# lewisjared/rscm

Hardware: AMD Instinct MI355X
Metric: ensemble-member-years/sec, two-layer 1750-2500 f64 (higher is better)
Workload: dtype f64

## Files before the change

### rscm_amd/csrc/two_layer.hip

```cpp
#include "two_layer_body.hpp"

namespace rscm {

namespace {

__device__ unsigned long long g_guard_counts[tl::kGuardKinds];

template <int MODE, bool LDS, bool STORE>
__global__ __launch_bounds__(kBlock) void two_layer_kernel(TwoLayerArgs a)
{
    extern __shared__ double lds_forcing[];
    if constexpr (LDS) {
        const int32_t len = a.step_end - a.step_begin;
        const int32_t total = a.n_scen * len;
        for (int32_t idx = threadIdx.x; idx < total; idx += kBlock) {
            const int32_t s = idx / len, k = idx - s * len;
            lds_forcing[idx] = a.forcing[(size_t)s * a.n_times + a.step_begin + a.src_off + k];
        }
        __syncthreads();
    }
    const int64_t i = (int64_t)blockIdx.x * kBlock + threadIdx.x;
    if (i >= a.n_members) return;
    const int32_t guard = tl::two_layer_body<MODE, LDS, STORE>(a, lds_forcing, i, a.step_begin, a.step_end);
    if constexpr (MODE == 0) {
        if (a.count_guards && (threadIdx.x & 63) == 0) atomicAdd(&g_guard_counts[guard], 1ull);
    }
}

template <int MODE, bool LDS>
__global__ __launch_bounds__(kBlock) void two_layer_ref_kernel(TwoLayerArgs a, TwoLayerRefArgs r)
{
    extern __shared__ double lds_forcing[];
    if constexpr (LDS) {
        const int32_t len = a.step_end - a.step_begin;
        const int32_t total = a.n_scen * len;
        for (int32_t idx = threadIdx.x; idx < total; idx += kBlock) {
            const int32_t s = idx / len, k = idx - s * len;
            lds_forcing[idx] = a.forcing[(size_t)s * a.n_times + a.step_begin + a.src_off + k];
        }
        __syncthreads();
    }
    const int64_t i = (int64_t)blockIdx.x * kBlock + threadIdx.x;
    if (i >= a.n_members) return;
    const int32_t guard = tl::two_layer_body<MODE, LDS, false, NoCache, true>(a, lds_forcing, i, a.step_begin, a.step_end, NoCache(), &r);
    if constexpr (MODE == 0) {
        if (a.count_guards && (threadIdx.x & 63) == 0) atomicAdd(&g_guard_counts[guard], 1ull);
    }
}

}


template <bool STORE>
static hipError_t launch_impl(const TwoLayerArgs& a, int mode, hipStream_t s)
{
    if (a.n_members <= 0) return hipSuccess;
    if (STORE && a.step_end <= a.step_begin) return hipSuccess;
    const size_t lds = a.lds_forcing ? (size_t)a.n_scen * (a.step_end - a.step_begin) * sizeof(double) : 0;
    const dim3 grid((unsigned)((a.n_members + kBlock - 1) / kBlock));
    void (*kern)(TwoLayerArgs) =
        mode == 0 ? (a.lds_forcing ? two_layer_kernel<0, true, STORE> : two_layer_kernel<0, false, STORE>)
                  : (a.lds_forcing ? two_layer_kernel<1, true, STORE> : two_layer_kernel<1, false, STORE>);
    if (lds > (size_t)kMaxStaticLds) {
        hipError_t e = hipFuncSetAttribute(reinterpret_cast<const void*>(kern),
                                           hipFuncAttributeMaxDynamicSharedMemorySize, (int)lds);
        if (e != hipSuccess) return e;
    }
    hipLaunchKernelGGL(kern, grid, dim3(kBlock), lds, s, a);
    return hipGetLastError();
}

hipError_t launch_two_layer(const TwoLayerArgs& a, int mode, hipStream_t s)
{
    return launch_impl<true>(a, mode, s);
}

hipError_t launch_two_layer_loglik(const TwoLayerArgs& a, int mode, hipStream_t s)
{
    return launch_impl<false>(a, mode, s);
}

hipError_t launch_two_layer_loglik_ref(const TwoLayerArgs& a, const TwoLayerRefArgs& r, int mode, hipStream_t s)
{
    if (a.n_members <= 0) return hipSuccess;
    const size_t lds = a.lds_forcing ? (size_t)a.n_scen * (a.step_end - a.step_begin) * sizeof(double) : 0;
    const dim3 grid((unsigned)((a.n_members + kBlock - 1) / kBlock));
    void (*kern)(TwoLayerArgs, TwoLayerRefArgs) =
        mode == 0 ? (a.lds_forcing ? two_layer_ref_kernel<0, true> : two_layer_ref_kernel<0, false>)
                  : (a.lds_forcing ? two_layer_ref_kernel<1, true> : two_layer_ref_kernel<1, false>);
    if (lds > (size_t)kMaxStaticLds) {
        hipError_t e = hipFuncSetAttribute(reinterpret_cast<const void*>(kern),
                                           hipFuncAttributeMaxDynamicSharedMemorySize, (int)lds);
        if (e != hipSuccess) return e;
    }
    hipLaunchKernelGGL(kern, grid, dim3(kBlock), lds, s, a, r);
    return hipGetLastError();
}

hipError_t two_layer_guard_counts(int64_t* out)
{
    unsigned long long c[tl::kGuardKinds] = {};
    hipError_t e = hipDeviceSynchronize();
    if (e == hipSuccess && out) e = hipMemcpyFromSymbol(c, HIP_SYMBOL(g_guard_counts), sizeof c);
    if (e != hipSuccess) return e;
    if (out)
        for (int k = 0; k < tl::kGuardKinds; ++k) out[k] = (int64_t)c[k];
    const unsigned long long zero[tl::kGuardKinds] = {};
    return hipMemcpyToSymbol(HIP_SYMBOL(g_guard_counts), zero, sizeof zero);
}

}
```

### rscm_amd/csrc/two_layer_body.hpp

```cpp
#pragma once

#include <type_traits>

#include "rk4_device.hpp"
#include "rscm_device.hpp"
#include "two_layer_box.hpp"
#include "two_layer_chunk_box.hpp"

namespace rscm {
namespace tl {

struct TLConst {
    double lambda0, a, eff_eta, eta, cs, cd, rcs, rcd;
};

template <bool SPEC, bool TAGS = SPEC>
__device__ __forceinline__ void rhs_exact(const TLConst& p, double erf, double ts, double td,
                                          double& dts, double& dtd, int32_t& acc)
{
    const double diff = ts - td;
    const double lambda_eff = p.lambda0 - p.a * ts;
    const double hx_s = p.eff_eta * diff;
    const double num_s = erf - lambda_eff * ts - hx_s;
    const double num_d = p.eta * diff;
    if constexpr (SPEC) {
        dts = spec_div(num_s, p.cs, p.rcs);
        dtd = spec_div(num_d, p.cd, p.rcd);
        if constexpr (TAGS) acc = max3_i32(acc, window_tag(num_s), window_tag(num_d));
    } else {
        dts = num_s / p.cs;
        dtd = num_d / p.cd;
    }
}

template <bool SPEC, bool TAGS = SPEC>
__device__ __forceinline__ void rk4_step_exact(const TLConst& p, double erf, double h,
                                               double half_step, double sixth, double& ts,
                                               double& td, int32_t& acc)
{
    double k1s, k1d, k2s, k2d, k3s, k3d, k4s, k4d;
    rhs_exact<SPEC, TAGS>(p, erf, ts, td, k1s, k1d, acc);
    rhs_exact<SPEC, TAGS>(p, erf, ts + k1s * half_step, td + k1d * half_step, k2s, k2d, acc);
    rhs_exact<SPEC, TAGS>(p, erf, ts + k2s * half_step, td + k2d * half_step, k3s, k3d, acc);
    rhs_exact<SPEC, TAGS>(p, erf, ts + k3s * h, td + k3d * h, k4s, k4d, acc);
    if constexpr (SPEC) {
        ts = rk4_combine_fused2(ts, k1s, k2s, k3s, k4s, sixth);
        td = rk4_combine_fused2(td, k1d, k2d, k3d, k4d, sixth);
    } else {
        ts = rk4_combine(ts, k1s, k2s, k3s, k4s, sixth);
        td = rk4_combine(td, k1d, k2d, k3d, k4d, sixth);
    }
}

namespace box {

constexpr double pow2(int e)
{
    double r = 1.0;
    for (; e > 0; --e) r *= 2.0;
    for (; e < 0; ++e) r *= 0.5;
    return r;
}

static_assert(kCsLo >= -128 && kCsHi <= 129 && kCdLo >= -128 && kCdHi <= 129, "heat-capacity boxes must lie in the divisor window");

constexpr uint32_t neg_edge(int lo) { return 0u - ((uint32_t)(1023 + lo) << 21); }
constexpr uint32_t span(int lo, int hi) { return (uint32_t)(hi - lo) << 21; }

__device__ __forceinline__ bool positive_in(double x, int lo, int hi)
{
    return x >= pow2(lo) && x < pow2(hi);
}

template <int lo = kForcingLo, int hi = kForcingHi>
__device__ __forceinline__ bool forcing_in(double f)
{
    return (__double_as_longlong(f) == 0) | (box_tag(f, neg_edge(lo)) < span(lo, hi));
}

__device__ __forceinline__ bool params_in(const TLConst& p, double h, double half_step)
{
    return positive_in(p.lambda0, kLambda0Lo, kLambda0Hi) &&
           (__double_as_longlong(p.a) == 0 || positive_in(p.a, kALo, kAHi)) &&
           positive_in(p.eff_eta, kEffEtaLo, kEffEtaHi) && positive_in(p.eta, kEtaLo, kEtaHi) &&
           positive_in(p.cs, kCsLo, kCsHi) && positive_in(p.cd, kCdLo, kCdHi) &&
           positive_in(h, kHLo, kHHi) && positive_in(half_step, kHLo, kHHi);
}

}

namespace chunk {

static_assert(kWideDivLo >= box::kCsLo && kWideDivHi <= box::kCdHi && kCsLo >= kWideDivLo && kCsHi <= kWideDivHi &&
                  kCdLo >= kWideDivLo && kCdHi <= kWideDivHi,
              "the chunk's heat capacities must lie in the wide window's divisor box");

__device__ __forceinline__ bool params_in(const TLConst& p, double h, double half_step, double sixth)
{
    using box::positive_in;
    return positive_in(p.lambda0, kLambda0Lo, kLambda0Hi) &&
           (__double_as_longlong(p.a) == 0 || positive_in(p.a, kALo, kAHi)) &&
           positive_in(p.eff_eta, kEffEtaLo, kEffEtaHi) && positive_in(p.eta, kEtaLo, kEtaHi) &&
           positive_in(p.cs, kCsLo, kCsHi) && positive_in(p.cd, kCdLo, kCdHi) &&
           positive_in(h, kHLo, kHHi) && positive_in(half_step, kHalfLo, kHalfHi) && positive_in(sixth, kSixthLo, kSixthHi);
}

}

constexpr int32_t kUnrolledSubSteps = 10;

struct TLFast {
    double l0, a, ee, ed;
};

__device__ __forceinline__ void rhs_fast(const TLFast& p, double erf_cs, double ts, double w, double& dts, double& dw)
{
    const double q = __builtin_fma(p.a, ts, -p.l0);
    const double t = __builtin_fma(q, ts, erf_cs);
    dts = __builtin_fma(-p.ee, w, t);
    dw = __builtin_fma(-p.ed, w, dts);
}

__device__ __forceinline__ void rk4_year_fast(const TLFast& p, double erf_cs, int32_t m, double h, double half_step, double third,
                                              double sixth, double& ts, double& td)
{
    double w = ts - td;
    for (int32_t s = 0; s < m; ++s) {
        double k1s, k1w, k2s, k2w, k3s, k3w, k4s, k4w;
        rhs_fast(p, erf_cs, ts, w, k1s, k1w);
        rhs_fast(p, erf_cs, __builtin_fma(k1s, half_step, ts), __builtin_fma(k1w, half_step, w), k2s, k2w);
        rhs_fast(p, erf_cs, __builtin_fma(k2s, half_step, ts), __builtin_fma(k2w, half_step, w), k3s, k3w);
        rhs_fast(p, erf_cs, __builtin_fma(k3s, h, ts), __builtin_fma(k3w, h, w), k4s, k4w);
        ts = __builtin_fma(k2s + k3s, third, __builtin_fma(k1s + k4s, sixth, ts));
        w = __builtin_fma(k2w + k3w, third, __builtin_fma(k1w + k4w, sixth, w));
    }
    td = ts - w;
}

__device__ __forceinline__ TLFast make_fast(double lambda0, double a, double efficacy, double eta, double cs, double cd, double& inv_cs)
{
    inv_cs = 1.0 / cs;
    TLFast p;
    p.l0 = lambda0 * inv_cs;
    p.a = a * inv_cs;
    p.ee = efficacy * eta * inv_cs;
    p.ed = eta / cd;
    return p;
}

struct LikAcc {
    double part_s = 0.0, part_d = 0.0;
    bool bad = false;
    int32_t oi = 0;
};

__device__ __forceinline__ void lik_consume(const TwoLayerArgs& a, LikAcc& L, int32_t row, double ts,
                                            double td)
{
    while (L.oi < a.n_obs && a.obs_tidx[L.oi] == row) {
        const bool deep = a.obs_is_deep[L.oi] != 0;
        const double m = deep ? td : ts;
        if (!is_finite(m)) L.bad = true;
        const double sigma = a.obs_sigma[L.oi];
        const double residual = a.obs_value[L.oi] - m;
        const double chi = (residual * residual) / (sigma * sigma);
        double l = -0.5 * chi;
        if (a.normalize) {
            l -= 0.5 * 1.8378770664093453;
            l -= log(sigma);
        }
        if (deep) L.part_d += l;
        else L.part_s += l;
        ++L.oi;
    }
}

struct LikRef {
    double sum_s = -0.0, sum_d = -0.0, b_s = 0.0, b_d = 0.0;
    bool have_s = false, have_d = false;
};

__device__ __forceinline__ double lik_term(const TwoLayerArgs& a, int32_t k, double m)
{
    const double sigma = a.obs_sigma[k];
    const double residual = a.obs_value[k] - m;
    const double chi = (residual * residual) / (sigma * sigma);
    double l = -0.5 * chi;
    if (a.normalize) {
        l -= 0.5 * 1.8378770664093453;
        l -= log(sigma);
    }
    return l;
}

__device__ __forceinline__ void lik_settle(const TwoLayerArgs& a, const TwoLayerRefArgs& r, LikAcc& L, bool deep, double sum, int32_t count,
                                           double& b, double& part, int64_t i, int64_t N)
{
    b = sum / (double)count;
    if (!is_finite(b)) L.bad = true;
    for (int32_t k = 0; k < L.oi; ++k) {
        const int32_t slot = r.obs_slot[k];
        if ((a.obs_is_deep[k] != 0) != deep || slot < 0) continue;
        part += lik_term(a, k, r.defer[(size_t)slot * N + i] - b);
    }
}

__device__ __forceinline__ void lik_consume_ref(const TwoLayerArgs& a, const TwoLayerRefArgs& r, LikAcc& L, LikRef& R, int32_t row,
                                                double ts, double td, int64_t i, int64_t N)
{
    auto reference_row = [&](int32_t v) {
        return r.on[v] && row >= r.begin[v] && row <= r.last[v] && (r.stride[v] == 1 || (row - r.begin[v]) % r.stride[v] == 0);
    };
    if (reference_row(0)) R.sum_s += ts;
    if (reference_row(1)) R.sum_d += td;
    while (L.oi < a.n_obs && a.obs_tidx[L.oi] == row) {
        const bool deep = a.obs_is_deep[L.oi] != 0;
        const double m = deep ? td : ts;
        if (!is_finite(m)) L.bad = true;
        const int32_t slot = r.obs_slot[L.oi];
        if (slot >= 0) {
            r.defer[(size_t)slot * N + i] = m;
        } else {
            const bool anomaly = deep ? r.on[1] != 0 : r.on[0] != 0;
            const double l = lik_term(a, L.oi, anomaly ? m - (deep ? R.b_d : R.b_s) : m);
            if (deep) L.part_d += l;
            else L.part_s += l;
        }
        ++L.oi;
    }
    if (r.on[0] && row == r.last[0]) {
        lik_settle(a, r, L, false, R.sum_s, r.count[0], R.b_s, L.part_s, i, N);
        R.have_s = true;
    }
    if (r.on[1] && row == r.last[1]) {
        lik_settle(a, r, L, true, R.sum_d, r.count[1], R.b_d, L.part_d, i, N);
        R.have_d = true;
    }
}

enum : int32_t { kGuardNumerators = 0, kGuardStates = 1, kGuardChunks = 2, kGuardKinds = 3 };

template <int MODE, bool LDS, bool STORE, class Cache = NoCache, bool REF = false>
__device__ __forceinline__ int32_t two_layer_body(const TwoLayerArgs& a, const double* lds_forcing, int64_t i, int32_t step_begin,
                                               int32_t step_end, const Cache& cache = Cache(), const TwoLayerRefArgs* ref = nullptr)
{
    static_assert(!(REF && STORE), "reference periods belong to the fused likelihood");
    const int32_t len = step_end - step_begin;
    const int64_t N = a.row_stride;

    const double lambda0 = cache.param(a.params, a.uniform_rows, 0, N, i);
    const double pa = cache.param(a.params, a.uniform_rows, 1, N, i);
    const double efficacy = cache.param(a.params, a.uniform_rows, 2, N, i);
    const double eta = cache.param(a.params, a.uniform_rows, 3, N, i);
    const double cs = cache.param(a.params, a.uniform_rows, 4, N, i);
    const double cd = cache.param(a.params, a.uniform_rows, 5, N, i);
    const int32_t scen = a.scen ? a.scen[i] : 0;
    const double* fglob = a.link ? a.link + (size_t)a.src_off * N + i : a.forcing + (size_t)scen * a.n_times + a.src_off;
    const size_t fstride = a.link ? (size_t)N : (size_t)1;
    const int32_t fl0 = scen * len - step_begin;
    auto forcing_at = [&](int32_t n) -> double {
        if constexpr (LDS) return lds_forcing[fl0 + n];
        else return fglob[(size_t)n * fstride];
    };
    auto forcing_first = [&]() -> double {
        if constexpr (Cache::kOn) {
            if (a.link && cache.has_link(0)) return cache.link(0);
        }
        return forcing_at(step_begin);
    };
    auto forcing_ahead = [&](int32_t n, int32_t np, double current) -> double {
        if constexpr (Cache::kOn) return n < np ? forcing_at(np) : current;
        else return forcing_at(np);
    };

    double ts = cache.state(0, a.ts + (size_t)step_begin * N + i);
    double td = cache.state(1, a.td + (size_t)step_begin * N + i);
    double* out_ts = a.ts + (size_t)(step_begin + 1) * N + i;
    double* out_td = a.td + (size_t)(step_begin + 1) * N + i;

    const double h = a.h;
    const double half_step = a.h_half;
    const double sixth = a.h_sixth;
    const int32_t last = step_end - 1;

    LikAcc lik;
    [[maybe_unused]] LikRef lik_ref;
    [[maybe_unused]] auto consume = [&](int32_t row) {
        if constexpr (REF) lik_consume_ref(a, *ref, lik, lik_ref, row, ts, td, i, N);
        else lik_consume(a, lik, row, ts, td);
    };
    if constexpr (!STORE) consume(step_begin);

    double erf_next = forcing_first();
    int32_t m_next = a.nsub[step_begin];

    int32_t guard = -1;
    if constexpr (MODE == 0) {
        TLConst p;
        p.lambda0 = lambda0;
        p.a = pa;
        p.eff_eta = efficacy * eta;
        p.eta = eta;
        p.cs = cs;
        p.cd = cd;
        const ConstDiv dcs = make_const_div(cs), dcd = make_const_div(cd);
        p.rcs = dcs.r;
        p.rcd = dcd.r;
        const int32_t acc0 = (dcs.ok && dcd.ok) ? (int32_t)0x80000000 : 0;
        const bool guard_states = __all(!a.numerator_guard && box::params_in(p, h, half_step));
        const bool guard_chunks = guard_states && __all(chunk::params_in(p, h, half_step, sixth));
        auto years = [&](auto guard) {
            constexpr int32_t kGuard = decltype(guard)::value;
            constexpr bool kStates = kGuard > 0;
            constexpr bool kChunks = kGuard > 1;
            for (int32_t n = step_begin; n < step_end; ++n) {
                const double erf = erf_next;
                const int32_t m = m_next;
                const int32_t np = n < last ? n + 1 : n;
                erf_next = forcing_ahead(n, np, erf_next);
                m_next = a.nsub[np];
                const double ts0 = ts, td0 = td;
                bool replay;
                if constexpr (kStates) {
                    int32_t no_tags = 0;
                    auto sub_step = [&](uint32_t& acc, uint32_t edge, bool tag) {
                        if (tag) acc = max3_u32(acc, box_tag(ts, edge), box_tag(td, edge));
                        rk4_step_exact<true, false>(p, erf, h, half_step, sixth, ts, td, no_tags);
                    };
                    if (kChunks && m == kUnrolledSubSteps) {
                        constexpr uint32_t kEdge = box::neg_edge(chunk::kStateLo), kSpan = box::span(chunk::kStateLo, chunk::kStateHi);
                        uint32_t acc = box::forcing_in<chunk::kForcingLo, chunk::kForcingHi>(erf) ? 0u : ~0u;
#pragma unroll
                        for (int32_t s = 0; s < kUnrolledSubSteps; ++s) sub_step(acc, kEdge, s % kGuard == 0);
                        replay = acc >= kSpan;
                    } else {
                        constexpr uint32_t kEdge = box::neg_edge(box::kStateLo), kSpan = box::span(box::kStateLo, box::kStateHi);
                        uint32_t acc = box::forcing_in(erf) ? 0u : ~0u;
                        if (m == kUnrolledSubSteps) {
#pragma unroll
                            for (int32_t s = 0; s < kUnrolledSubSteps; ++s) sub_step(acc, kEdge, true);
                        } else {
                            for (int32_t s = 0; s < m; ++s) sub_step(acc, kEdge, true);
                        }
                        replay = acc >= kSpan;
                    }
                } else {
                    int32_t acc = acc0;
                    for (int32_t s = 0; s < m; ++s) rk4_step_exact<true>(p, erf, h, half_step, sixth, ts, td, acc);
                    replay = acc >= 0;
                }
                const bool settled = (ts0 != ts0) || (td0 != td0);
                if (__builtin_expect(replay && !settled, 0)) {
                    ts = ts0;
                    td = td0;
                    int32_t unused = 0;
                    for (int32_t s = 0; s < m; ++s) rk4_step_exact<false>(p, erf, h, half_step, sixth, ts, td, unused);
                }
                if constexpr (STORE) {
                    *out_ts = ts;
                    *out_td = td;
                    cache.put(0, ts);
                    cache.put(1, td);
                    out_ts += N;
                    out_td += N;
                } else {
                    consume(n + 1);
                }
            }
        };
        if (guard_chunks) years(std::integral_constant<int32_t, chunk::kChunkSubSteps>());
        else if (guard_states) years(std::integral_constant<int32_t, 1>());
        else years(std::integral_constant<int32_t, 0>());
        guard = guard_chunks ? kGuardChunks : guard_states ? kGuardStates : kGuardNumerators;
    } else {
        double inv_cs;
        const TLFast p = make_fast(lambda0, pa, efficacy, eta, cs, cd, inv_cs);
        const double third = h / 3.0;
        for (int32_t n = step_begin; n < step_end; ++n) {
            const double erf = erf_next * inv_cs;
            const int32_t m = m_next;
            const int32_t np = n < last ? n + 1 : n;
            erf_next = forcing_ahead(n, np, erf_next);
            m_next = a.nsub[np];
            rk4_year_fast(p, erf, m, h, half_step, third, sixth, ts, td);
            if constexpr (STORE) {
                *out_ts = ts;
                *out_td = td;
                cache.put(0, ts);
                cache.put(1, td);
                out_ts += N;
                out_td += N;
            } else {
                consume(n + 1);
            }
        }
    }
    if (cache.last_step()) a.status[i] = (is_finite(ts) && is_finite(td)) ? 0 : 1;
    if constexpr (!STORE) {
        if (lik.oi < a.n_obs) lik.bad = true;
        if constexpr (REF) {
            if ((ref->on[0] && !lik_ref.have_s) || (ref->on[1] && !lik_ref.have_d)) lik.bad = true;
        }
        const double total = a.first_is_deep ? (0.0 + lik.part_d) + lik.part_s
                                             : (0.0 + lik.part_s) + lik.part_d;
        a.loglik[i] = lik.bad ? -__builtin_inf() : total;
    }
    return guard;
}

}
}
```

Baseline: 34.99 billion.

## Read uniform forcing via scalar loads and unroll year loop in pairs

When all members share one forcing series, the kernels now skip LDS staging and read forcing and substep counts through scalar (constant address space) loads. The year loop is restructured to process two years per iteration with lookahead prefetch, and adds a lean path that drops the forcing range check once upcoming years are known to be in range. Replay of out-of-box steps becomes wave-uniform via ballot, and output stores use a wave-base pointer plus lane offset. This adds template instantiations and code complexity, and relies on forcing and nsub being safe to read through scalar loads.

Result: no change. 34.95 billion, median of 2 (-0.1%).

```diff
diff --git a/rscm_amd/csrc/two_layer.hip b/rscm_amd/csrc/two_layer.hip
--- a/rscm_amd/csrc/two_layer.hip
+++ b/rscm_amd/csrc/two_layer.hip
@@ -6,22 +6,36 @@
 
 __device__ unsigned long long g_guard_counts[tl::kGuardKinds];
 
+__host__ __device__ inline bool uniform_forcing(const TwoLayerArgs& a)
+{
+    return a.scen == nullptr && a.n_scen == 1 && a.link == nullptr && a.n_times < (1 << 28);
+}
+
+__device__ __forceinline__ void stage_forcing(const TwoLayerArgs& a, double* lds_forcing)
+{
+    const int32_t len = a.step_end - a.step_begin;
+    const int32_t total = a.n_scen * len;
+    for (int32_t idx = threadIdx.x; idx < total; idx += kBlock) {
+        const int32_t s = idx / len, k = idx - s * len;
+        lds_forcing[idx] = a.forcing[(size_t)s * a.n_times + a.step_begin + a.src_off + k];
+    }
+    __syncthreads();
+}
+
 template <int MODE, bool LDS, bool STORE>
 __global__ __launch_bounds__(kBlock) void two_layer_kernel(TwoLayerArgs a)
 {
     extern __shared__ double lds_forcing[];
-    if constexpr (LDS) {
-        const int32_t len = a.step_end - a.step_begin;
-        const int32_t total = a.n_scen * len;
-        for (int32_t idx = threadIdx.x; idx < total; idx += kBlock) {
-            const int32_t s = idx / len, k = idx - s * len;
-            lds_forcing[idx] = a.forcing[(size_t)s * a.n_times + a.step_begin + a.src_off + k];
-        }
-        __syncthreads();
+    const int64_t i = (int64_t)blockIdx.x * kBlock + threadIdx.x;
+    int32_t guard;
+    if (uniform_forcing(a)) {
+        if (i >= a.n_members) return;
+        guard = tl::two_layer_body<MODE, false, STORE, NoCache, false, true>(a, nullptr, i, a.step_begin, a.step_end);
+    } else {
+        if constexpr (LDS) stage_forcing(a, lds_forcing);
+        if (i >= a.n_members) return;
+        guard = tl::two_layer_body<MODE, LDS, STORE>(a, lds_forcing, i, a.step_begin, a.step_end);
     }
-    const int64_t i = (int64_t)blockIdx.x * kBlock + threadIdx.x;
-    if (i >= a.n_members) return;
-    const int32_t guard = tl::two_layer_body<MODE, LDS, STORE>(a, lds_forcing, i, a.step_begin, a.step_end);
     if constexpr (MODE == 0) {
         if (a.count_guards && (threadIdx.x & 63) == 0) atomicAdd(&g_guard_counts[guard], 1ull);
     }
@@ -31,18 +45,16 @@
 __global__ __launch_bounds__(kBlock) void two_layer_ref_kernel(TwoLayerArgs a, TwoLayerRefArgs r)
 {
     extern __shared__ double lds_forcing[];
-    if constexpr (LDS) {
-        const int32_t len = a.step_end - a.step_begin;
-        const int32_t total = a.n_scen * len;
-        for (int32_t idx = threadIdx.x; idx < total; idx += kBlock) {
-            const int32_t s = idx / len, k = idx - s * len;
-            lds_forcing[idx] = a.forcing[(size_t)s * a.n_times + a.step_begin + a.src_off + k];
-        }
-        __syncthreads();
+    const int64_t i = (int64_t)blockIdx.x * kBlock + threadIdx.x;
+    int32_t guard;
+    if (uniform_forcing(a)) {
+        if (i >= a.n_members) return;
+        guard = tl::two_layer_body<MODE, false, false, NoCache, true, true>(a, nullptr, i, a.step_begin, a.step_end, NoCache(), &r);
+    } else {
+        if constexpr (LDS) stage_forcing(a, lds_forcing);
+        if (i >= a.n_members) return;
+        guard = tl::two_layer_body<MODE, LDS, false, NoCache, true>(a, lds_forcing, i, a.step_begin, a.step_end, NoCache(), &r);
     }
-    const int64_t i = (int64_t)blockIdx.x * kBlock + threadIdx.x;
-    if (i >= a.n_members) return;
-    const int32_t guard = tl::two_layer_body<MODE, LDS, false, NoCache, true>(a, lds_forcing, i, a.step_begin, a.step_end, NoCache(), &r);
     if constexpr (MODE == 0) {
         if (a.count_guards && (threadIdx.x & 63) == 0) atomicAdd(&g_guard_counts[guard], 1ull);
     }
@@ -56,7 +68,7 @@
 {
     if (a.n_members <= 0) return hipSuccess;
     if (STORE && a.step_end <= a.step_begin) return hipSuccess;
-    const size_t lds = a.lds_forcing ? (size_t)a.n_scen * (a.step_end - a.step_begin) * sizeof(double) : 0;
+    const size_t lds = (a.lds_forcing && !uniform_forcing(a)) ? (size_t)a.n_scen * (a.step_end - a.step_begin) * sizeof(double) : 0;
     const dim3 grid((unsigned)((a.n_members + kBlock - 1) / kBlock));
     void (*kern)(TwoLayerArgs) =
         mode == 0 ? (a.lds_forcing ? two_layer_kernel<0, true, STORE> : two_layer_kernel<0, false, STORE>)
@@ -83,7 +95,7 @@
 hipError_t launch_two_layer_loglik_ref(const TwoLayerArgs& a, const TwoLayerRefArgs& r, int mode, hipStream_t s)
 {
     if (a.n_members <= 0) return hipSuccess;
-    const size_t lds = a.lds_forcing ? (size_t)a.n_scen * (a.step_end - a.step_begin) * sizeof(double) : 0;
+    const size_t lds = (a.lds_forcing && !uniform_forcing(a)) ? (size_t)a.n_scen * (a.step_end - a.step_begin) * sizeof(double) : 0;
     const dim3 grid((unsigned)((a.n_members + kBlock - 1) / kBlock));
     void (*kern)(TwoLayerArgs, TwoLayerRefArgs) =
         mode == 0 ? (a.lds_forcing ? two_layer_ref_kernel<0, true> : two_layer_ref_kernel<0, false>)
diff --git a/rscm_amd/csrc/two_layer_body.hpp b/rscm_amd/csrc/two_layer_body.hpp
--- a/rscm_amd/csrc/two_layer_body.hpp
+++ b/rscm_amd/csrc/two_layer_body.hpp
@@ -76,6 +76,15 @@
 __device__ __forceinline__ bool forcing_in(double f)
 {
     return (__double_as_longlong(f) == 0) | (box_tag(f, neg_edge(lo)) < span(lo, hi));
+}
+
+template <int lo = kForcingLo, int hi = kForcingHi>
+__device__ __forceinline__ uint32_t forcing_acc_uniform(double f)
+{
+    const uint64_t bits = (uint64_t)__double_as_longlong(f);
+    const uint32_t tag = ((uint32_t)(bits >> 32) << 1) + neg_edge(lo);
+    const uint32_t outside = tag < span(lo, hi) ? 0u : ~0u;
+    return bits == 0 ? 0u : outside;
 }
 
 __device__ __forceinline__ bool params_in(const TLConst& p, double h, double half_step)
@@ -240,11 +249,18 @@
 
 enum : int32_t { kGuardNumerators = 0, kGuardStates = 1, kGuardChunks = 2, kGuardKinds = 3 };
 
-template <int MODE, bool LDS, bool STORE, class Cache = NoCache, bool REF = false>
+__device__ __forceinline__ int64_t first_lane(int64_t v)
+{
+    const uint32_t lo = __builtin_amdgcn_readfirstlane((uint32_t)v), hi = __builtin_amdgcn_readfirstlane((uint32_t)((uint64_t)v >> 32));
+    return (int64_t)(((uint64_t)hi << 32) | lo);
+}
+
+template <int MODE, bool LDS, bool STORE, class Cache = NoCache, bool REF = false, bool UNIFORM = false>
 __device__ __forceinline__ int32_t two_layer_body(const TwoLayerArgs& a, const double* lds_forcing, int64_t i, int32_t step_begin,
                                                int32_t step_end, const Cache& cache = Cache(), const TwoLayerRefArgs* ref = nullptr)
 {
     static_assert(!(REF && STORE), "reference periods belong to the fused likelihood");
+    static_assert(!(UNIFORM && (LDS || Cache::kOn)), "the uniform forcing is read from the table, by the stand-alone kernels");
     const int32_t len = step_end - step_begin;
     const int64_t N = a.row_stride;
 
@@ -254,13 +270,21 @@
     const double eta = cache.param(a.params, a.uniform_rows, 3, N, i);
     const double cs = cache.param(a.params, a.uniform_rows, 4, N, i);
     const double cd = cache.param(a.params, a.uniform_rows, 5, N, i);
-    const int32_t scen = a.scen ? a.scen[i] : 0;
-    const double* fglob = a.link ? a.link + (size_t)a.src_off * N + i : a.forcing + (size_t)scen * a.n_times + a.src_off;
-    const size_t fstride = a.link ? (size_t)N : (size_t)1;
+    const int32_t scen = (!UNIFORM && a.scen) ? a.scen[i] : 0;
+    const double* fglob = (!UNIFORM && a.link) ? a.link + (size_t)a.src_off * N + i : a.forcing + (size_t)scen * a.n_times + a.src_off;
+    const size_t fstride = (!UNIFORM && a.link) ? (size_t)N : (size_t)1;
     const int32_t fl0 = scen * len - step_begin;
+    typedef const __attribute__((address_space(4))) char* scalar_bytes;
+    [[maybe_unused]] const scalar_bytes funi = (scalar_bytes)(uintptr_t)(a.forcing + a.src_off);
+    const scalar_bytes nuni = (scalar_bytes)(uintptr_t)a.nsub;
     auto forcing_at = [&](int32_t n) -> double {
-        if constexpr (LDS) return lds_forcing[fl0 + n];
+        if constexpr (UNIFORM) return *(const volatile __attribute__((address_space(4))) double*)(funi + ((uint32_t)n << 3));
+        else if constexpr (LDS) return lds_forcing[fl0 + n];
         else return fglob[(size_t)n * fstride];
+    };
+    auto nsub = [&](int32_t n) -> int32_t {
+        if constexpr (UNIFORM) return *(const volatile __attribute__((address_space(4))) int32_t*)(nuni + ((uint32_t)n << 2));
+        else return ((const __attribute__((address_space(4))) int32_t*)nuni)[n];
     };
     auto forcing_first = [&]() -> double {
         if constexpr (Cache::kOn) {
@@ -268,15 +292,14 @@
         }
         return forcing_at(step_begin);
     };
-    auto forcing_ahead = [&](int32_t n, int32_t np, double current) -> double {
-        if constexpr (Cache::kOn) return n < np ? forcing_at(np) : current;
-        else return forcing_at(np);
-    };
 
     double ts = cache.state(0, a.ts + (size_t)step_begin * N + i);
     double td = cache.state(1, a.td + (size_t)step_begin * N + i);
-    double* out_ts = a.ts + (size_t)(step_begin + 1) * N + i;
-    double* out_td = a.td + (size_t)(step_begin + 1) * N + i;
+    const int64_t i0 = first_lane(i);
+    [[maybe_unused]] uint32_t lane_off = (uint32_t)(i - i0) * (uint32_t)sizeof(double);
+    [[maybe_unused]] char* row_ts = reinterpret_cast<char*>(a.ts + (size_t)(step_begin + 1) * N + i0);
+    [[maybe_unused]] char* row_td = reinterpret_cast<char*>(a.td + (size_t)(step_begin + 1) * N + i0);
+    const size_t row_bytes = (size_t)N * sizeof(double);
 
     const double h = a.h;
     const double half_step = a.h_half;
@@ -291,8 +314,70 @@
     };
     if constexpr (!STORE) consume(step_begin);
 
-    double erf_next = forcing_first();
-    int32_t m_next = a.nsub[step_begin];
+    auto finish_year = [&](int32_t n) __attribute__((always_inline)) {
+        if constexpr (STORE) {
+            asm volatile("" : "+v"(lane_off));
+            *reinterpret_cast<double*>(row_ts + lane_off) = ts;
+            *reinterpret_cast<double*>(row_td + lane_off) = td;
+            cache.put(0, ts);
+            cache.put(1, td);
+            row_ts += row_bytes;
+            row_td += row_bytes;
+        } else {
+            consume(n + 1);
+        }
+    };
+
+    auto run_years = [&](auto&& year, auto has_lean, auto&& lean_ok) __attribute__((always_inline)) {
+        constexpr bool kLean = decltype(has_lean)::value;
+        double erf_a = forcing_first();
+        int32_t m_a = nsub(step_begin);
+        if constexpr (Cache::kOn || (MODE == 1 && !STORE && !LDS && !UNIFORM)) {
+            for (int32_t n = step_begin; n < step_end; ++n) {
+                const double erf = erf_a;
+                const int32_t m = m_a;
+                const int32_t np = n < last ? n + 1 : n;
+                if (n < np) erf_a = forcing_at(np);
+                m_a = nsub(np);
+                year(n, erf, m, std::false_type());
+            }
+        } else {
+            asm volatile("" : "+v"(ts), "+v"(td));
+            const int32_t n1 = step_begin < last ? step_begin + 1 : step_begin;
+            double erf_b = forcing_at(n1);
+            int32_t m_b = nsub(n1);
+            int32_t n = step_begin;
+            auto pair = [&](auto lean) __attribute__((always_inline)) {
+                year(n, erf_a, m_a, lean);
+                const int32_t na = n + 2 < last ? n + 2 : last, nb = n + 3 < last ? n + 3 : last;
+                erf_a = forcing_at(na);
+                m_a = nsub(na);
+                const double erf_next = forcing_at(nb);
+                const int32_t m_next = nsub(nb);
+                year(n + 1, erf_b, m_b, lean);
+                erf_b = erf_next;
+                m_b = m_next;
+            };
+            if constexpr (kLean) {
+                auto lean_ahead = [&]() { return lean_ok(erf_a, m_a) && lean_ok(erf_b, m_b); };
+                while (n < last && !lean_ahead()) {
+                    year(n, erf_a, m_a, std::false_type());
+                    ++n;
+                    erf_a = erf_b;
+                    m_a = m_b;
+                    const int32_t nb = n + 1 < last ? n + 1 : last;
+                    erf_b = forcing_at(nb);
+                    m_b = nsub(nb);
+                }
+                while (n < last && __builtin_expect(lean_ahead(), 1)) {
+                    pair(std::true_type());
+                    n += 2;
+                }
+            }
+            for (; n < last; n += 2) pair(std::false_type());
+            if (n < step_end) year(n, erf_a, m_a, std::false_type());
+        }
+    };
 
     int32_t guard = -1;
     if constexpr (MODE == 0) {
@@ -313,12 +398,12 @@
             constexpr int32_t kGuard = decltype(guard)::value;
             constexpr bool kStates = kGuard > 0;
             constexpr bool kChunks = kGuard > 1;
-            for (int32_t n = step_begin; n < step_end; ++n) {
-                const double erf = erf_next;
-                const int32_t m = m_next;
-                const int32_t np = n < last ? n + 1 : n;
-                erf_next = forcing_ahead(n, np, erf_next);
-                m_next = a.nsub[np];
+            auto lean_ok = [&](double erf, int32_t m) -> bool {
+                const uint32_t tag = ((uint32_t)((uint64_t)__double_as_longlong(erf) >> 32) << 1) + box::neg_edge(chunk::kForcingLo);
+                return (tag < box::span(chunk::kForcingLo, chunk::kForcingHi) ? m : -1) == kUnrolledSubSteps;
+            };
+            run_years([&](int32_t n, double erf, int32_t m, auto lean) __attribute__((always_inline)) {
+                constexpr bool kLeanYear = decltype(lean)::value;
                 const double ts0 = ts, td0 = td;
                 bool replay;
                 if constexpr (kStates) {
@@ -327,46 +412,52 @@
                         if (tag) acc = max3_u32(acc, box_tag(ts, edge), box_tag(td, edge));
                         rk4_step_exact<true, false>(p, erf, h, half_step, sixth, ts, td, no_tags);
                     };
-                    if (kChunks && m == kUnrolledSubSteps) {
-                        constexpr uint32_t kEdge = box::neg_edge(chunk::kStateLo), kSpan = box::span(chunk::kStateLo, chunk::kStateHi);
-                        uint32_t acc = box::forcing_in<chunk::kForcingLo, chunk::kForcingHi>(erf) ? 0u : ~0u;
+                    uint32_t acc, span;
+                    if constexpr (kLeanYear) {
+                        constexpr uint32_t kEdge = box::neg_edge(chunk::kStateLo);
+                        acc = 0u;
 #pragma unroll
                         for (int32_t s = 0; s < kUnrolledSubSteps; ++s) sub_step(acc, kEdge, s % kGuard == 0);
-                        replay = acc >= kSpan;
+                        span = box::span(chunk::kStateLo, chunk::kStateHi);
+                    } else
+                    if (kChunks && __builtin_expect(m == kUnrolledSubSteps, 1)) {
+                        constexpr uint32_t kEdge = box::neg_edge(chunk::kStateLo);
+                        if constexpr (UNIFORM) acc = box::forcing_acc_uniform<chunk::kForcingLo, chunk::kForcingHi>(erf);
+                        else acc = box::forcing_in<chunk::kForcingLo, chunk::kForcingHi>(erf) ? 0u : ~0u;
+#pragma unroll
+                        for (int32_t s = 0; s < kUnrolledSubSteps; ++s) sub_step(acc, kEdge, s % kGuard == 0);
+                        span = box::span(chunk::kStateLo, chunk::kStateHi);
                     } else {
-                        constexpr uint32_t kEdge = box::neg_edge(box::kStateLo), kSpan = box::span(box::kStateLo, box::kStateHi);
-                        uint32_t acc = box::forcing_in(erf) ? 0u : ~0u;
-                        if (m == kUnrolledSubSteps) {
+                        constexpr uint32_t kEdge = box::neg_edge(box::kStateLo);
+                        if constexpr (UNIFORM) acc = box::forcing_acc_uniform(erf);
+                        else acc = box::forcing_in(erf) ? 0u : ~0u;
+                        if (__builtin_expect(m == kUnrolledSubSteps, !kChunks)) {
 #pragma unroll
                             for (int32_t s = 0; s < kUnrolledSubSteps; ++s) sub_step(acc, kEdge, true);
                         } else {
                             for (int32_t s = 0; s < m; ++s) sub_step(acc, kEdge, true);
                         }
-                        replay = acc >= kSpan;
+                        span = box::span(box::kStateLo, box::kStateHi);
                     }
+                    replay = acc >= span;
                 } else {
                     int32_t acc = acc0;
                     for (int32_t s = 0; s < m; ++s) rk4_step_exact<true>(p, erf, h, half_step, sixth, ts, td, acc);
                     replay = acc >= 0;
                 }
-                const bool settled = (ts0 != ts0) || (td0 != td0);
-                if (__builtin_expect(replay && !settled, 0)) {
-                    ts = ts0;
-                    td = td0;
-                    int32_t unused = 0;
-                    for (int32_t s = 0; s < m; ++s) rk4_step_exact<false>(p, erf, h, half_step, sixth, ts, td, unused);
+                if (__builtin_expect(__builtin_amdgcn_ballot_w64(replay) != 0, 0)) {
+                    const bool settled = (ts0 != ts0) || (td0 != td0);
+                    const bool redo = replay && !settled;
+                    if (__builtin_amdgcn_ballot_w64(redo) != 0) {
+                        double rs = ts0, rd = td0;
+                        int32_t unused = 0;
+                        for (int32_t s = 0; s < m; ++s) rk4_step_exact<false>(p, erf, h, half_step, sixth, rs, rd, unused);
+                        ts = redo ? rs : ts;
+                        td = redo ? rd : td;
+                    }
                 }
-                if constexpr (STORE) {
-                    *out_ts = ts;
-                    *out_td = td;
-                    cache.put(0, ts);
-                    cache.put(1, td);
-                    out_ts += N;
-                    out_td += N;
-                } else {
-                    consume(n + 1);
-                }
-            }
+                finish_year(n);
+            }, std::integral_constant<bool, UNIFORM && kChunks>(), lean_ok);
         };
         if (guard_chunks) years(std::integral_constant<int32_t, chunk::kChunkSubSteps>());
         else if (guard_states) years(std::integral_constant<int32_t, 1>());
@@ -376,24 +467,10 @@
         double inv_cs;
         const TLFast p = make_fast(lambda0, pa, efficacy, eta, cs, cd, inv_cs);
         const double third = h / 3.0;
-        for (int32_t n = step_begin; n < step_end; ++n) {
-            const double erf = erf_next * inv_cs;
-            const int32_t m = m_next;
-            const int32_t np = n < last ? n + 1 : n;
-            erf_next = forcing_ahead(n, np, erf_next);
-            m_next = a.nsub[np];
-            rk4_year_fast(p, erf, m, h, half_step, third, sixth, ts, td);
-            if constexpr (STORE) {
-                *out_ts = ts;
-                *out_td = td;
-                cache.put(0, ts);
-                cache.put(1, td);
-                out_ts += N;
-                out_td += N;
-            } else {
-                consume(n + 1);
-            }
-        }
+        run_years([&](int32_t n, double erf, int32_t m, auto) __attribute__((always_inline)) {
+            rk4_year_fast(p, erf * inv_cs, m, h, half_step, third, sixth, ts, td);
+            finish_year(n);
+        }, std::false_type(), 0);
     }
     if (cache.last_step()) a.status[i] = (is_finite(ts) && is_finite(td)) ? 0 : 1;
     if constexpr (!STORE) {
```
